# Ighina/MultimodalTopicSegmentation

Measured on NVIDIA B200. Metric: segmented sentences/sec, higher is better.
Workload: dtype f32

## Files before the change

multimodaltopicsegmentation_b200/csrc/lstm_rec_h3.cu:

```cuda
#include <cooperative_groups.h>
#include <cuda_fp16.h>
#include <stdlib.h>

#include "cluster_utils.cuh"
#include "tcgen05_utils.cuh"

namespace cg = cooperative_groups;

namespace mts {

constexpr int HR_NB = 16;
constexpr int HR_SUB_THREADS = 160;
constexpr int HR_EPI = 128;
constexpr int HR_PIECE_BYTES = 4 * HR_NB * 128;
constexpr int HR_B_BYTES = 2 * HR_PIECE_BYTES;
constexpr int HR_ACT_FLOATS = 4 * HR_NB * 32;
constexpr int HR_TMEM_COLS = 512;
constexpr int HR_W2_COL = 128;
constexpr int HR_ACC_COL = 256;
constexpr int HR_SUB_BYTES = 2 * HR_B_BYTES + HR_ACT_FLOATS * 4 + 1024;
constexpr int HR_HEAD_BYTES = 1024;
static_assert(HR_SUB_BYTES % 1024 == 0, "SWIZZLE_128B operand buffers need 1024-byte alignment");
template <int NT>
constexpr int hr_smem() {
  return (HR_HEAD_BYTES + NT * HR_SUB_BYTES + 1024) > 120 * 1024 ? (HR_HEAD_BYTES + NT * HR_SUB_BYTES + 1024) : 120 * 1024;
}

__host__ __device__ constexpr uint32_t idesc_f16(int M, int N) {
  return (1u << 4) | ((uint32_t)(N >> 3) << 17) | ((uint32_t)(M >> 4) << 24);
}

__device__ __forceinline__ uint32_t h2_bits(float first, float second) {
  const __half2 h = __floats2half2_rn(first, second);
  return *reinterpret_cast<const uint32_t *>(&h);
}
__device__ __forceinline__ float2 h2_floats(uint32_t bits) {
  return __half22float2(*reinterpret_cast<const __half2 *>(&bits));
}
__device__ __forceinline__ void st_async_v4u(uint32_t raddr, uint4 v, uint32_t rbar) {
  asm volatile("st.async.weak.shared::cluster.mbarrier::complete_tx::bytes.v4.b32 [%0], {%1, %2, %3, %4}, [%5];" ::"r"(raddr),
               "r"(v.x), "r"(v.y), "r"(v.z), "r"(v.w), "r"(rbar)
               : "memory");
}
__device__ __forceinline__ void tmem_st16u(uint32_t taddr, const uint32_t (&v)[16]) {
  asm volatile(
      "tcgen05.st.sync.aligned.32x32b.x16.b32 [%0], "
      "{%1, %2, %3, %4, %5, %6, %7, %8, %9, %10, %11, %12, %13, %14, %15, %16};" ::"r"(taddr),
      "r"(v[0]), "r"(v[1]), "r"(v[2]), "r"(v[3]), "r"(v[4]), "r"(v[5]), "r"(v[6]), "r"(v[7]), "r"(v[8]), "r"(v[9]), "r"(v[10]),
      "r"(v[11]), "r"(v[12]), "r"(v[13]), "r"(v[14]), "r"(v[15])
      : "memory");
}

__device__ __forceinline__ void umma_f16_ts_p(uint32_t d_tmem, uint32_t a_tmem, uint32_t b_lo, uint32_t b_hi, uint32_t idesc,
                                              uint32_t acc) {
  asm volatile(
      "{\n\t.reg .pred p;\n\t.reg .b64 bd;\n\t"
      "setp.ne.b32 p, %5, 0;\n\t"
      "mov.b64 bd, {%2, %3};\n\t"
      "tcgen05.mma.cta_group::1.kind::f16 [%0], [%1], bd, %4, p;\n\t}" ::"r"(d_tmem),
      "r"(a_tmem), "r"(b_lo), "r"(b_hi), "r"(idesc), "r"(acc)
      : "memory");
}

constexpr int HR_PROF_STEPS = 4, HR_PROF_SLOTS = 16;
__device__ long long *g_hr_prof = nullptr;
#define HR_STAMP(slot)                                                                     \
  do {                                                                                     \
    if (prof && s >= 8 && s < 8 + HR_PROF_STEPS) prof[(s - 8) * HR_PROF_SLOTS + (slot)] = clock64(); \
  } while (0)

template <bool SAVE, int NT, bool BF16>
__global__ void __cluster_dims__(kCluster, 1, 1) __launch_bounds__(HR_SUB_THREADS * NT, 1)
    lstm_fwd_h3_kernel(const float *__restrict__ gx, const float *__restrict__ w_hh, const int32_t *__restrict__ lengths,
                       const int32_t *__restrict__ order, int B, int T, int n_enc, int n_tiles, int ept,
                       float *__restrict__ y, float *__restrict__ gates, float *__restrict__ y_corr) {
  constexpr bool bf16_mode = BF16;
  extern __shared__ uint8_t smem_raw[];
  uint8_t *smem = reinterpret_cast<uint8_t *>((reinterpret_cast<uintptr_t>(smem_raw) + 1023) & ~(uintptr_t)1023);
  const int tid = threadIdx.x, lane = tid & 31;
  const int warp = __shfl_sync(0xffffffffu, tid >> 5, 0);
  const int sub = (NT == 2 && warp >= 5) ? 1 : 0;
  const int wr = warp - 5 * sub;

  float *rscale_s = reinterpret_cast<float *>(smem);
  uint32_t *tmem_slot = reinterpret_cast<uint32_t *>(smem + 512);
  uint8_t *sub_base = smem + HR_HEAD_BYTES + sub * HR_SUB_BYTES;
  uint8_t *bbuf = sub_base;
  float *act = reinterpret_cast<float *>(bbuf + 2 * HR_B_BYTES);
  uint64_t *bars = reinterpret_cast<uint64_t *>(act + HR_ACT_FLOATS);
  uint64_t *h_full = bars;
  uint64_t *acc_full = bars + 16;
  int *len_s = reinterpret_cast<int *>(bars + 18);
  int *bq_s = len_s + HR_NB;

  cg::cluster_group cluster = cg::this_cluster();
  const uint32_t rank = cluster.block_rank();
  const int n_clusters = gridDim.x / kCluster;
  const int groups = (n_tiles + NT - 1) / NT;
  const int n_items = groups * 2 * n_enc;
  const int ycols = n_enc * 2 * kH;

  if (wr == 0 && lane == 0) {
    for (int i = 0; i < 4; ++i) tc::bar_init(tc::s_u32(&h_full[i]), 1);
    tc::bar_init(tc::s_u32(acc_full), 1);
    asm volatile("fence.mbarrier_init.release.cluster;" ::: "memory");
  }
  if (warp == 0) tc::tmem_alloc<HR_TMEM_COLS>(tc::s_u32(tmem_slot));
  tc::tc_fence_before();
  __syncthreads();
  tc::tc_fence_after();
  const uint32_t tmem_base = *tmem_slot;
  const uint32_t acc_col = HR_ACC_COL + 16 * sub;

  uint32_t ph_h = 0, ph_acc = 0;

  const int et = (wr - 1) * 32 + lane;
  const int q = warp & 3;
  const int cj = et & 7, ce = et >> 3;

  int cur_dir = -1, cur_enc = -1;
  long long *prof = (blockIdx.x == 0 && (tid == 0 || tid == 32)) ? g_hr_prof : nullptr;

  for (int item = blockIdx.x / kCluster; item < n_items; item += n_clusters) {
    const int tile = (item % groups) * NT + sub;
    const int dir = (item / groups) & 1;
    const int enc = item / (2 * groups);
    const float *W = w_hh + ((size_t)enc * 2 + dir) * 4 * kH * kH;

    if (dir != cur_dir || enc != cur_enc) {
      if (sub == 0 && wr >= 1) {
        const float *wrow = W + (size_t)(q * kH + rank * kUnits + lane) * kH;
        float mx = 0.0f;
#pragma unroll 8
        for (int i = 0; i < kH / 4; ++i) {
          const float4 x = __ldg(reinterpret_cast<const float4 *>(wrow) + i);
          mx = fmaxf(fmaxf(mx, fmaxf(fabsf(x.x), fabsf(x.y))), fmaxf(fabsf(x.z), fabsf(x.w)));
        }
        const int ex = (int)((__float_as_uint(mx) >> 23) & 0xFFu);
        int sexp = ex == 0 ? 0 : 127 + 13 - ex;
        sexp = sexp > 110 ? 110 : sexp;
        const float sc = __uint_as_float((uint32_t)(127 + sexp) << 23);
        rscale_s[q * 32 + lane] = __uint_as_float((uint32_t)(127 - sexp) << 23);
        const uint32_t trow = tmem_base + ((uint32_t)(q * 32) << 16);
#pragma unroll 1
        for (int kk = 0; kk < 8; ++kk) {
          const int src_blk = ((int)rank - kk) & 7;
          uint32_t w1[16], w2[16];
#pragma unroll
          for (int i = 0; i < 8; ++i) {
            const float4 x = __ldg(reinterpret_cast<const float4 *>(wrow + src_blk * 32) + i);
            const float a = x.x * sc, b = x.y * sc, c = x.z * sc, d = x.w * sc;
            if (bf16_mode) {
              w1[2 * i] = bf16x2_bits(a, b);
              w1[2 * i + 1] = bf16x2_bits(c, d);
              w2[2 * i] = w2[2 * i + 1] = 0u;
            } else {
              w1[2 * i] = h2_bits(a, b);
              w1[2 * i + 1] = h2_bits(c, d);
              const float2 f0 = h2_floats(w1[2 * i]), f1 = h2_floats(w1[2 * i + 1]);
              w2[2 * i] = h2_bits(a - f0.x, b - f0.y);
              w2[2 * i + 1] = h2_bits(c - f1.x, d - f1.y);
            }
          }
          tmem_st16u(trow + (uint32_t)(kk * 16), w1);
          tmem_st16u(trow + (uint32_t)(HR_W2_COL + kk * 16), w2);
        }
        tc::tmem_wait_st();
      }
      cur_dir = dir;
      cur_enc = enc;
    }
    const int st = tid - sub * HR_SUB_THREADS;
    if (st < HR_NB) {
      const int slot = tile * ept + st;
      const int bq = (tile < n_tiles && st < ept && slot < B) ? (order ? order[slot] : slot) : -1;
      bq_s[st] = bq;
      len_s[st] = (bq >= 0) ? min(max(lengths[bq], 0), T) : 0;
    }
    for (int idx = st; idx < 2 * HR_B_BYTES / 16; idx += HR_SUB_THREADS)
      reinterpret_cast<float4 *>(bbuf)[idx] = make_float4(0.f, 0.f, 0.f, 0.f);
    tc::fence_proxy_async();
    tc::tc_fence_before();
    __syncthreads();
    tc::tc_fence_after();
    int nsteps = 0;
#pragma unroll
    for (int e = 0; e < HR_NB; ++e) nsteps = max(nsteps, len_s[e]);
    cluster.sync();

    const size_t gx_enc = (size_t)enc * B * T * 8 * kH;

    if (wr == 0) {
      constexpr uint32_t idesc = bf16_mode ? tc::idesc_bf16(128, HR_NB) : idesc_f16(128, HR_NB);
      const uint32_t tb = __shfl_sync(0xffffffffu, tmem_base, 0);
      const uint32_t d_tmem = tb + acc_col;
      const bool leader = tc::elect_one();
      const uint64_t dfull = tc::desc_sw128(tc::s_u32(bbuf));
      const uint32_t dlo0 = __shfl_sync(0xffffffffu, (uint32_t)dfull, 0), dhi = (uint32_t)(dfull >> 32);
      const uint32_t half_tx = (uint32_t)(4 * ept * (bf16_mode ? 64 : 128));
      for (int s = 0; s < nsteps; ++s) {
        const int p = s & 1;
        HR_STAMP(0);
        if (leader && s + 1 < nsteps) {
          tc::bar_expect_tx(tc::s_u32(&h_full[(p ^ 1) * 2 + 0]), half_tx);
          tc::bar_expect_tx(tc::s_u32(&h_full[(p ^ 1) * 2 + 1]), half_tx);
        }
        const uint32_t dlo = dlo0 + (uint32_t)(p * (HR_B_BYTES >> 4));
#pragma unroll
        for (int g = 0; g < 2; ++g) {
          if (s > 0) tc::bar_wait_wd(tc::s_u32(&h_full[p * 2 + g]), (ph_h >> p) & 1u);
          HR_STAMP(1 + g);
          tc::tc_fence_after();
          if (leader) {
#pragma unroll
            for (int i = 4 * g; i < 4 * g + 4; ++i) {
#pragma unroll
              for (int k = 0; k < 2; ++k) {
                const uint32_t d1 = dlo + (uint32_t)(((i >> 1) * (HR_NB * 128) + (i & 1) * 64 + k * 32) >> 4);
                const uint32_t d2 = d1 + (uint32_t)(HR_PIECE_BYTES >> 4);
                const uint32_t a1 = tb + (uint32_t)(16 * i + 8 * k), a2 = a1 + HR_W2_COL;
                umma_f16_ts_p(d_tmem, a1, d1, dhi, idesc, (i | k) != 0);
                if (!bf16_mode) {
                  umma_f16_ts_p(d_tmem, a2, d1, dhi, idesc, 1);
                  umma_f16_ts_p(d_tmem, a1, d2, dhi, idesc, 1);
                }
              }
            }
          }
          HR_STAMP(3 + g);
        }
        if (s > 0) ph_h ^= 1u << p;
        if (leader) tc::umma_commit(tc::s_u32(acc_full));
        __syncwarp();
        HR_STAMP(5);
      }
    } else {
      const int gcol = dir * 4 * kH + q * kH + (int)rank * kUnits + lane;
      const float rs = rscale_s[q * 32 + lane];
      float gxn[HR_NB];
#pragma unroll
      for (int e = 0; e < HR_NB; ++e) {
        const int len = len_s[e];
        gxn[e] = 0.0f;
        if (len > 0) {
          const int t0 = dir ? len - 1 : 0;
          gxn[e] = __ldg(gx + gx_enc + ((size_t)bq_s[e] * T + t0) * 8 * kH + gcol);
        }
      }
      float c[4] = {0.f, 0.f, 0.f, 0.f};
      const int my_len = len_s[ce], my_b = bq_s[ce];
      const size_t ycol = (size_t)enc * 2 * kH + dir * kH + rank * kUnits + 4 * cj;
      const size_t gate_base = ((size_t)enc * 2 + dir) * B;
      const int piece = cj & 1, chunk = cj >> 1;
      uint32_t raddr[kCluster], rbar[kCluster];
#pragma unroll
      for (int i = 0; i < kCluster; ++i) {
        const uint32_t r = (rank + i) & 7;
        const uint32_t off = (uint32_t)(piece * HR_PIECE_BYTES + (i >> 1) * (HR_NB * 128) + ce * 128 +
                                        ((((i & 1) * 4 + chunk) ^ (ce & 7)) << 4));
        raddr[i] = mapa(tc::s_u32(bbuf) + off, r);
        rbar[i] = mapa(tc::s_u32(&h_full[i >> 2]), r);
      }
      const bool sender = ce < ept && !(bf16_mode && piece);

      for (int s = 0; s < nsteps; ++s) {
        const int p = s & 1;
        float gxc[HR_NB];
#pragma unroll
        for (int e = 0; e < HR_NB; ++e) {
          gxc[e] = gxn[e];
          const int len = len_s[e];
          if (s + 1 < len) {
            const int tn = dir ? len - 2 - s : s + 1;
            gxn[e] = __ldg(gx + gx_enc + ((size_t)bq_s[e] * T + tn) * 8 * kH + gcol);
          }
        }
        tc::bar_wait_wd(tc::s_u32(acc_full), ph_acc); ph_acc ^= 1;
        HR_STAMP(10);
        tc::tc_fence_after();
        float pre[HR_NB];
        tc::tmem_ld16(tmem_base + ((uint32_t)(q * 32) << 16) + acc_col, pre);
        tc::tc_fence_before();
        HR_STAMP(11);
        const float zs = (q == 2) ? -2.0f * 1.4426950408889634f : -1.4426950408889634f;
        const float oa = (q == 2) ? 2.0f : 1.0f, ob = (q == 2) ? -1.0f : 0.0f;
#define HR_ACT(NCOL)                                                          \
  _Pragma("unroll") for (int e = 0; e < (NCOL); ++e) {                        \
    const float z = fmaf(pre[e], rs, gxc[e]);                                 \
    const float sg = __fdividef(1.0f, 1.0f + exp2f(z * zs));                  \
    act[(q * HR_NB + e) * 32 + lane] = fmaf(sg, oa, ob);                      \
  }
        if (ept > 14) { HR_ACT(16) } else if (ept > 12) { HR_ACT(14) } else if (ept > 10) { HR_ACT(12) } else if (ept > 8) { HR_ACT(10) }
        else if (ept > 6) { HR_ACT(8) } else if (ept > 4) { HR_ACT(6) } else if (ept > 2) { HR_ACT(4) } else { HR_ACT(2) }
#undef HR_ACT
        if (sub == 0) asm volatile("bar.sync 1, 128;" ::: "memory");
        else asm volatile("bar.sync 2, 128;" ::: "memory");
        HR_STAMP(12);
        const float4 ig = *reinterpret_cast<const float4 *>(act + (0 * HR_NB + ce) * 32 + 4 * cj);
        const float4 fg = *reinterpret_cast<const float4 *>(act + (1 * HR_NB + ce) * 32 + 4 * cj);
        const float4 gg = *reinterpret_cast<const float4 *>(act + (2 * HR_NB + ce) * 32 + 4 * cj);
        const float4 og = *reinterpret_cast<const float4 *>(act + (3 * HR_NB + ce) * 32 + 4 * cj);
        float4 hn = make_float4(0.f, 0.f, 0.f, 0.f);
        if (s < my_len) {
          c[0] = fmaf(fg.x, c[0], ig.x * gg.x); c[1] = fmaf(fg.y, c[1], ig.y * gg.y);
          c[2] = fmaf(fg.z, c[2], ig.z * gg.z); c[3] = fmaf(fg.w, c[3], ig.w * gg.w);
          hn = make_float4(og.x * tanh_fast(c[0]), og.y * tanh_fast(c[1]), og.z * tanh_fast(c[2]), og.w * tanh_fast(c[3]));
        }
        HR_STAMP(13);
        if (s + 1 < nsteps) {
          uint32_t p1a, p1b, p2a = 0u, p2b = 0u;
          if (bf16_mode) {
            p1a = bf16x2_bits(hn.x, hn.y);
            p1b = bf16x2_bits(hn.z, hn.w);
          } else {
            p1a = h2_bits(hn.x, hn.y);
            p1b = h2_bits(hn.z, hn.w);
            const float2 f0 = h2_floats(p1a), f1 = h2_floats(p1b);
            p2a = h2_bits(hn.x - f0.x, hn.y - f0.y);
            p2b = h2_bits(hn.z - f1.x, hn.w - f1.y);
          }
          const uint32_t ga = piece ? p1a : p2a, gb = piece ? p1b : p2b;
          const uint32_t ra = __shfl_xor_sync(0xffffffffu, ga, 1), rb = __shfl_xor_sync(0xffffffffu, gb, 1);
          const uint4 gran = piece ? make_uint4(ra, rb, p2a, p2b) : make_uint4(p1a, p1b, ra, rb);
          if (sender) {
            const uint32_t boff = (uint32_t)((p ^ 1) * HR_B_BYTES), moff = (uint32_t)((p ^ 1) * 16);
#pragma unroll
            for (int r = 0; r < kCluster; ++r) st_async_v4u(raddr[r] + boff, gran, rbar[r] + moff);
          }
        }
        HR_STAMP(14);
        if (s < my_len) {
          const int t = dir ? my_len - 1 - s : s;
          *reinterpret_cast<float4 *>(y + ((size_t)my_b * T + t) * ycols + ycol) = hn;
          if (y_corr) corr_store4(y_corr + ((size_t)my_b * T + t) * ycols, (int)ycol, hn, 0);
          if (SAVE) {
            float *gs = gates + ((gate_base + my_b) * T + t) * 5 * kH + rank * kUnits + 4 * cj;
            *reinterpret_cast<float4 *>(gs) = ig;
            *reinterpret_cast<float4 *>(gs + kH) = fg;
            *reinterpret_cast<float4 *>(gs + 2 * kH) = gg;
            *reinterpret_cast<float4 *>(gs + 3 * kH) = og;
            *reinterpret_cast<float4 *>(gs + 4 * kH) = make_float4(c[0], c[1], c[2], c[3]);
          }
        }
      }
      if (my_b >= 0)
        for (int t = my_len; t < T; ++t) {
          const float4 z = make_float4(0.f, 0.f, 0.f, 0.f);
          *reinterpret_cast<float4 *>(y + ((size_t)my_b * T + t) * ycols + ycol) = z;
          if (y_corr) corr_store4(y_corr + ((size_t)my_b * T + t) * ycols, (int)ycol, z, 0);
        }
    }
    tc::tc_fence_before();
    __syncthreads();
    cluster.sync();
  }
  tc::tc_fence_before();
  __syncthreads();
  if (warp == 0) {
    tc::tc_fence_after();
    tc::tmem_dealloc<HR_TMEM_COLS>(tmem_base);
  }
}

template <typename K>
static int h3_max_active_clusters(K kernel, int threads, int smem) {
  cudaLaunchConfig_t cfg = {};
  cfg.gridDim = dim3(kCluster * 64);
  cfg.blockDim = dim3(threads);
  cfg.dynamicSmemBytes = smem;
  cudaLaunchAttribute attr;
  attr.id = cudaLaunchAttributeClusterDimension;
  attr.val.clusterDim.x = kCluster;
  attr.val.clusterDim.y = 1;
  attr.val.clusterDim.z = 1;
  cfg.attrs = &attr;
  cfg.numAttrs = 1;
  int n = 0;
  if (cudaOccupancyMaxActiveClusters(&n, kernel, &cfg) != cudaSuccess || n < 1) {
    cudaGetLastError();
    n = 8;
  }
  return n;
}

}

using namespace mts;

extern "C" int mts_debug_rec_profile_h3(long long *buf) {
  MTS_CUDA(cudaMemcpyToSymbol(g_hr_prof, &buf, sizeof(buf)));
  return 0;
}

template <bool BF16>
static int launch_h3(const float *gx, const float *w_hh, const int32_t *lengths, const int32_t *order, int n_enc, int B, int T,
                     float *y, float *gates, float *y_corr, cudaStream_t st) {
  MTS_PER_DEVICE(int, cap);
  if (!cap) {
    MTS_CUDA(cudaFuncSetAttribute(lstm_fwd_h3_kernel<false, 1, BF16>, cudaFuncAttributeMaxDynamicSharedMemorySize, hr_smem<1>()));
    MTS_CUDA(cudaFuncSetAttribute(lstm_fwd_h3_kernel<true, 1, BF16>, cudaFuncAttributeMaxDynamicSharedMemorySize, hr_smem<1>()));
    MTS_CUDA(cudaFuncSetAttribute(lstm_fwd_h3_kernel<false, 2, BF16>, cudaFuncAttributeMaxDynamicSharedMemorySize, hr_smem<2>()));
    MTS_CUDA(cudaFuncSetAttribute(lstm_fwd_h3_kernel<true, 2, BF16>, cudaFuncAttributeMaxDynamicSharedMemorySize, hr_smem<2>()));
    cap = h3_max_active_clusters(lstm_fwd_h3_kernel<false, 2, BF16>, 2 * HR_SUB_THREADS, hr_smem<2>());
  }
  int ept = HR_NB;
  {
    const int per_dir = cap / (2 * n_enc);
    if (per_dir >= 1 && (B + HR_NB - 1) / HR_NB <= per_dir) {
      const int want = (B + per_dir - 1) / per_dir;
      ept = want < 1 ? 1 : (want > HR_NB ? HR_NB : want);
    }
  }
  static const char *force_ept = getenv("MTS_REC_EPT");
  if (force_ept && atoi(force_ept) >= 1 && atoi(force_ept) <= HR_NB) ept = atoi(force_ept);
  const int n_tiles = (B + ept - 1) / ept;
  const int items1 = n_tiles * 2 * n_enc;
  static const char *force = getenv("MTS_REC_NT");
  const bool two = force ? (force[0] == '2') : (items1 > cap);
  static const char *pair_env = getenv("MTS_REC_PAIR");
  if (pair_env ? (pair_env[0] == '1') : two)
    return mts_lstm_rec_fwd_h3p(gx, w_hh, lengths, order, n_enc, B, T, kH, y, gates, y_corr, BF16 ? 1 : 0, (void *)st);
  if (!two) {
    const unsigned grid = (unsigned)((items1 < cap ? items1 : cap) * kCluster);
    if (gates) lstm_fwd_h3_kernel<true, 1, BF16><<<grid, HR_SUB_THREADS, hr_smem<1>(), st>>>(gx, w_hh, lengths, order, B, T, n_enc, n_tiles, ept, y, gates, y_corr);
    else lstm_fwd_h3_kernel<false, 1, BF16><<<grid, HR_SUB_THREADS, hr_smem<1>(), st>>>(gx, w_hh, lengths, order, B, T, n_enc, n_tiles, ept, y, gates, y_corr);
  } else {
    const int items2 = ((n_tiles + 1) / 2) * 2 * n_enc;
    const unsigned grid = (unsigned)((items2 < cap ? items2 : cap) * kCluster);
    if (gates) lstm_fwd_h3_kernel<true, 2, BF16><<<grid, 2 * HR_SUB_THREADS, hr_smem<2>(), st>>>(gx, w_hh, lengths, order, B, T, n_enc, n_tiles, ept, y, gates, y_corr);
    else lstm_fwd_h3_kernel<false, 2, BF16><<<grid, 2 * HR_SUB_THREADS, hr_smem<2>(), st>>>(gx, w_hh, lengths, order, B, T, n_enc, n_tiles, ept, y, gates, y_corr);
  }
  MTS_LAUNCH_CHECK();
  return 0;
}

extern "C" int mts_lstm_rec_fwd_h3(const float *gx, const float *w_hh, const int32_t *lengths, const int32_t *order, int n_enc,
                                   int B, int T, int H, float *y, float *gates, float *y_corr, int precision, void *stream) {
  MTS_REQUIRE(gx && w_hh && lengths && y, MTS_E_BADARG, "lstm_rec_fwd_h3: null pointer");
  MTS_REQUIRE(n_enc >= 1 && B > 0 && T > 0, MTS_E_BADARG, "lstm_rec_fwd_h3: bad shape");
  MTS_REQUIRE(H == kH, MTS_E_UNSUPPORTED, "lstm_rec_fwd_h3: the tensor-core recurrence serves H == 256");
  MTS_REQUIRE(precision == 0 || precision == 1, MTS_E_BADARG, "lstm_rec_fwd_h3: precision must be 0 (fp16 x3) or 1 (bf16)");
  MTS_REQUIRE(!y_corr || n_enc == 1, MTS_E_UNSUPPORTED, "lstm_rec_fwd_h3: the fused correction operand needs n_enc == 1");
  MTS_REQUIRE((((uintptr_t)y | (uintptr_t)gx | (uintptr_t)w_hh) & 15) == 0, MTS_E_BADARG,
              "lstm_rec_fwd_h3: buffers must be 16-byte aligned");
  cudaStream_t st = (cudaStream_t)stream;
  return precision ? launch_h3<true>(gx, w_hh, lengths, order, n_enc, B, T, y, gates, y_corr, st)
                   : launch_h3<false>(gx, w_hh, lengths, order, n_enc, B, T, y, gates, y_corr, st);
}
```

Measured before the change: 18.58 million.

## Split LSTM recurrence epilogue across eight warps for single-tile pipeline

Adds an eight-warp epilogue variant in which each group of four warps handles half of the batch columns. It loads eight TMEM columns instead of sixteen and remaps the cell-update lanes across the larger warp set, which shortens the per-step serial activation and cell-update work on the recurrence's critical path. The variant is used in the single-tile path whenever there are at least three elements per tile, or when forced by an environment variable. In exchange the block is larger and uses a wider named barrier, and the column interleave adds indexing complexity.

```diff
diff --git a/multimodaltopicsegmentation_b200/csrc/lstm_rec_h3.cu b/multimodaltopicsegmentation_b200/csrc/lstm_rec_h3.cu
--- a/multimodaltopicsegmentation_b200/csrc/lstm_rec_h3.cu
+++ b/multimodaltopicsegmentation_b200/csrc/lstm_rec_h3.cu
@@ -10,8 +10,7 @@
 namespace mts {
 
 constexpr int HR_NB = 16;
-constexpr int HR_SUB_THREADS = 160;
-constexpr int HR_EPI = 128;
+constexpr int HR_EPI8_MIN_EPT = 3;
 constexpr int HR_PIECE_BYTES = 4 * HR_NB * 128;
 constexpr int HR_B_BYTES = 2 * HR_PIECE_BYTES;
 constexpr int HR_ACT_FLOATS = 4 * HR_NB * 32;
@@ -42,6 +41,20 @@
                "r"(v.x), "r"(v.y), "r"(v.z), "r"(v.w), "r"(rbar)
                : "memory");
 }
+__device__ __forceinline__ void tmem_ld8(uint32_t taddr, float (&v)[8]) {
+  uint32_t r[8];
+  asm volatile("tcgen05.ld.sync.aligned.32x32b.x8.b32 {%0, %1, %2, %3, %4, %5, %6, %7}, [%8];"
+               : "=r"(r[0]), "=r"(r[1]), "=r"(r[2]), "=r"(r[3]), "=r"(r[4]), "=r"(r[5]), "=r"(r[6]), "=r"(r[7])
+               : "r"(taddr)
+               : "memory");
+  asm volatile("tcgen05.wait::ld.sync.aligned;" ::: "memory");
+#pragma unroll
+  for (int i = 0; i < 8; ++i) v[i] = __uint_as_float(r[i]);
+}
+template <int HALVES>
+__device__ __forceinline__ int hr_col(int e) {
+  return (e % HALVES) * (HR_NB / HALVES) + e / HALVES;
+}
 __device__ __forceinline__ void tmem_st16u(uint32_t taddr, const uint32_t (&v)[16]) {
   asm volatile(
       "tcgen05.st.sync.aligned.32x32b.x16.b32 [%0], "
@@ -69,18 +82,22 @@
     if (prof && s >= 8 && s < 8 + HR_PROF_STEPS) prof[(s - 8) * HR_PROF_SLOTS + (slot)] = clock64(); \
   } while (0)
 
-template <bool SAVE, int NT, bool BF16>
-__global__ void __cluster_dims__(kCluster, 1, 1) __launch_bounds__(HR_SUB_THREADS * NT, 1)
+template <bool SAVE, int NT, bool BF16, int EW>
+__global__ void __cluster_dims__(kCluster, 1, 1) __launch_bounds__(32 * (1 + EW) * NT, 1)
     lstm_fwd_h3_kernel(const float *__restrict__ gx, const float *__restrict__ w_hh, const int32_t *__restrict__ lengths,
                        const int32_t *__restrict__ order, int B, int T, int n_enc, int n_tiles, int ept,
                        float *__restrict__ y, float *__restrict__ gates, float *__restrict__ y_corr) {
+  static_assert(EW == 4 || (EW == 8 && NT == 1), "eight epilogue warps only with one tile pipeline");
   constexpr bool bf16_mode = BF16;
+  constexpr int SUBT = 32 * (1 + EW);
+  constexpr int HALVES = EW / 4;
+  constexpr int CPW = HR_NB / HALVES;
   extern __shared__ uint8_t smem_raw[];
   uint8_t *smem = reinterpret_cast<uint8_t *>((reinterpret_cast<uintptr_t>(smem_raw) + 1023) & ~(uintptr_t)1023);
   const int tid = threadIdx.x, lane = tid & 31;
   const int warp = __shfl_sync(0xffffffffu, tid >> 5, 0);
-  const int sub = (NT == 2 && warp >= 5) ? 1 : 0;
-  const int wr = warp - 5 * sub;
+  const int sub = (NT == 2 && warp > EW) ? 1 : 0;
+  const int wr = warp - (1 + EW) * sub;
 
   float *rscale_s = reinterpret_cast<float *>(smem);
   uint32_t *tmem_slot = reinterpret_cast<uint32_t *>(smem + 512);
@@ -114,9 +131,8 @@
 
   uint32_t ph_h = 0, ph_acc = 0;
 
-  const int et = (wr - 1) * 32 + lane;
   const int q = warp & 3;
-  const int cj = et & 7, ce = et >> 3;
+  const int col0 = ((wr - 1) >> 2) * CPW;
 
   int cur_dir = -1, cur_enc = -1;
   long long *prof = (blockIdx.x == 0 && (tid == 0 || tid == 32)) ? g_hr_prof : nullptr;
@@ -128,7 +144,7 @@
     const float *W = w_hh + ((size_t)enc * 2 + dir) * 4 * kH * kH;
 
     if (dir != cur_dir || enc != cur_enc) {
-      if (sub == 0 && wr >= 1) {
+      if (sub == 0 && wr >= 1 && wr <= 4) {
         const float *wrow = W + (size_t)(q * kH + rank * kUnits + lane) * kH;
         float mx = 0.0f;
 #pragma unroll 8
@@ -170,14 +186,14 @@
       cur_dir = dir;
       cur_enc = enc;
     }
-    const int st = tid - sub * HR_SUB_THREADS;
+    const int st = tid - sub * SUBT;
     if (st < HR_NB) {
       const int slot = tile * ept + st;
       const int bq = (tile < n_tiles && st < ept && slot < B) ? (order ? order[slot] : slot) : -1;
-      bq_s[st] = bq;
-      len_s[st] = (bq >= 0) ? min(max(lengths[bq], 0), T) : 0;
+      bq_s[hr_col<HALVES>(st)] = bq;
+      len_s[hr_col<HALVES>(st)] = (bq >= 0) ? min(max(lengths[bq], 0), T) : 0;
     }
-    for (int idx = st; idx < 2 * HR_B_BYTES / 16; idx += HR_SUB_THREADS)
+    for (int idx = st; idx < 2 * HR_B_BYTES / 16; idx += SUBT)
       reinterpret_cast<float4 *>(bbuf)[idx] = make_float4(0.f, 0.f, 0.f, 0.f);
     tc::fence_proxy_async();
     tc::tc_fence_before();
@@ -237,49 +253,54 @@
     } else {
       const int gcol = dir * 4 * kH + q * kH + (int)rank * kUnits + lane;
       const float rs = rscale_s[q * 32 + lane];
-      float gxn[HR_NB];
-#pragma unroll
-      for (int e = 0; e < HR_NB; ++e) {
-        const int len = len_s[e];
+      float gxn[CPW];
+#pragma unroll
+      for (int e = 0; e < CPW; ++e) {
+        const int len = len_s[col0 + e];
         gxn[e] = 0.0f;
         if (len > 0) {
           const int t0 = dir ? len - 1 : 0;
-          gxn[e] = __ldg(gx + gx_enc + ((size_t)bq_s[e] * T + t0) * 8 * kH + gcol);
+          gxn[e] = __ldg(gx + gx_enc + ((size_t)bq_s[col0 + e] * T + t0) * 8 * kH + gcol);
         }
       }
+      const int piece = lane & 1, chunk = (lane >> 1) & 3, cj = 2 * chunk + piece;
+      const int ce = (lane >> 3) * EW + ((wr - 1 - chunk * ept) & (EW - 1));
+      const bool cell = ce < ept;
+      const int row = cell ? hr_col<HALVES>(ce) : 0;
       float c[4] = {0.f, 0.f, 0.f, 0.f};
-      const int my_len = len_s[ce], my_b = bq_s[ce];
+      const int my_len = cell ? len_s[row] : 0, my_b = cell ? bq_s[row] : -1;
       const size_t ycol = (size_t)enc * 2 * kH + dir * kH + rank * kUnits + 4 * cj;
       const size_t gate_base = ((size_t)enc * 2 + dir) * B;
-      const int piece = cj & 1, chunk = cj >> 1;
       uint32_t raddr[kCluster], rbar[kCluster];
 #pragma unroll
       for (int i = 0; i < kCluster; ++i) {
         const uint32_t r = (rank + i) & 7;
-        const uint32_t off = (uint32_t)(piece * HR_PIECE_BYTES + (i >> 1) * (HR_NB * 128) + ce * 128 +
-                                        ((((i & 1) * 4 + chunk) ^ (ce & 7)) << 4));
+        const uint32_t off = (uint32_t)(piece * HR_PIECE_BYTES + (i >> 1) * (HR_NB * 128) + row * 128 +
+                                        ((((i & 1) * 4 + chunk) ^ (row & 7)) << 4));
         raddr[i] = mapa(tc::s_u32(bbuf) + off, r);
         rbar[i] = mapa(tc::s_u32(&h_full[i >> 2]), r);
       }
-      const bool sender = ce < ept && !(bf16_mode && piece);
+      const bool sender = cell && !(bf16_mode && piece);
+      const int ncol = (ept + HALVES - 1 - col0 / CPW) / HALVES;
 
       for (int s = 0; s < nsteps; ++s) {
         const int p = s & 1;
-        float gxc[HR_NB];
-#pragma unroll
-        for (int e = 0; e < HR_NB; ++e) {
+        float gxc[CPW];
+#pragma unroll
+        for (int e = 0; e < CPW; ++e) {
           gxc[e] = gxn[e];
-          const int len = len_s[e];
+          const int len = len_s[col0 + e];
           if (s + 1 < len) {
             const int tn = dir ? len - 2 - s : s + 1;
-            gxn[e] = __ldg(gx + gx_enc + ((size_t)bq_s[e] * T + tn) * 8 * kH + gcol);
+            gxn[e] = __ldg(gx + gx_enc + ((size_t)bq_s[col0 + e] * T + tn) * 8 * kH + gcol);
           }
         }
         tc::bar_wait_wd(tc::s_u32(acc_full), ph_acc); ph_acc ^= 1;
         HR_STAMP(10);
         tc::tc_fence_after();
-        float pre[HR_NB];
-        tc::tmem_ld16(tmem_base + ((uint32_t)(q * 32) << 16) + acc_col, pre);
+        float pre[CPW];
+        if constexpr (CPW == 16) tc::tmem_ld16(tmem_base + ((uint32_t)(q * 32) << 16) + acc_col, pre);
+        else tmem_ld8(tmem_base + ((uint32_t)(q * 32) << 16) + acc_col + col0, pre);
         tc::tc_fence_before();
         HR_STAMP(11);
         const float zs = (q == 2) ? -2.0f * 1.4426950408889634f : -1.4426950408889634f;
@@ -288,20 +309,24 @@
   _Pragma("unroll") for (int e = 0; e < (NCOL); ++e) {                        \
     const float z = fmaf(pre[e], rs, gxc[e]);                                 \
     const float sg = __fdividef(1.0f, 1.0f + exp2f(z * zs));                  \
-    act[(q * HR_NB + e) * 32 + lane] = fmaf(sg, oa, ob);                      \
-  }
-        if (ept > 14) { HR_ACT(16) } else if (ept > 12) { HR_ACT(14) } else if (ept > 10) { HR_ACT(12) } else if (ept > 8) { HR_ACT(10) }
-        else if (ept > 6) { HR_ACT(8) } else if (ept > 4) { HR_ACT(6) } else if (ept > 2) { HR_ACT(4) } else { HR_ACT(2) }
+    act[(q * HR_NB + col0 + e) * 32 + lane] = fmaf(sg, oa, ob);               \
+  }
+        if constexpr (CPW == 16) {
+          if (ncol > 14) { HR_ACT(16) } else if (ncol > 12) { HR_ACT(14) } else if (ncol > 10) { HR_ACT(12) } else if (ncol > 8) { HR_ACT(10) }
+          else if (ncol > 6) { HR_ACT(8) } else if (ncol > 4) { HR_ACT(6) } else if (ncol > 2) { HR_ACT(4) } else { HR_ACT(2) }
+        } else {
+          if (ncol > 6) { HR_ACT(8) } else if (ncol > 4) { HR_ACT(6) } else if (ncol > 2) { HR_ACT(4) } else if (ncol > 0) { HR_ACT(2) }
+        }
 #undef HR_ACT
-        if (sub == 0) asm volatile("bar.sync 1, 128;" ::: "memory");
-        else asm volatile("bar.sync 2, 128;" ::: "memory");
+        asm volatile("bar.sync %0, %1;" ::"r"(1 + sub), "n"(32 * EW) : "memory");
         HR_STAMP(12);
-        const float4 ig = *reinterpret_cast<const float4 *>(act + (0 * HR_NB + ce) * 32 + 4 * cj);
-        const float4 fg = *reinterpret_cast<const float4 *>(act + (1 * HR_NB + ce) * 32 + 4 * cj);
-        const float4 gg = *reinterpret_cast<const float4 *>(act + (2 * HR_NB + ce) * 32 + 4 * cj);
-        const float4 og = *reinterpret_cast<const float4 *>(act + (3 * HR_NB + ce) * 32 + 4 * cj);
+        float4 ig, fg, gg, og;
         float4 hn = make_float4(0.f, 0.f, 0.f, 0.f);
         if (s < my_len) {
+          ig = *reinterpret_cast<const float4 *>(act + (0 * HR_NB + row) * 32 + 4 * cj);
+          fg = *reinterpret_cast<const float4 *>(act + (1 * HR_NB + row) * 32 + 4 * cj);
+          gg = *reinterpret_cast<const float4 *>(act + (2 * HR_NB + row) * 32 + 4 * cj);
+          og = *reinterpret_cast<const float4 *>(act + (3 * HR_NB + row) * 32 + 4 * cj);
           c[0] = fmaf(fg.x, c[0], ig.x * gg.x); c[1] = fmaf(fg.y, c[1], ig.y * gg.y);
           c[2] = fmaf(fg.z, c[2], ig.z * gg.z); c[3] = fmaf(fg.w, c[3], ig.w * gg.w);
           hn = make_float4(og.x * tanh_fast(c[0]), og.y * tanh_fast(c[1]), og.z * tanh_fast(c[2]), og.w * tanh_fast(c[3]));
@@ -397,11 +422,13 @@
                      float *y, float *gates, float *y_corr, cudaStream_t st) {
   MTS_PER_DEVICE(int, cap);
   if (!cap) {
-    MTS_CUDA(cudaFuncSetAttribute(lstm_fwd_h3_kernel<false, 1, BF16>, cudaFuncAttributeMaxDynamicSharedMemorySize, hr_smem<1>()));
-    MTS_CUDA(cudaFuncSetAttribute(lstm_fwd_h3_kernel<true, 1, BF16>, cudaFuncAttributeMaxDynamicSharedMemorySize, hr_smem<1>()));
-    MTS_CUDA(cudaFuncSetAttribute(lstm_fwd_h3_kernel<false, 2, BF16>, cudaFuncAttributeMaxDynamicSharedMemorySize, hr_smem<2>()));
-    MTS_CUDA(cudaFuncSetAttribute(lstm_fwd_h3_kernel<true, 2, BF16>, cudaFuncAttributeMaxDynamicSharedMemorySize, hr_smem<2>()));
-    cap = h3_max_active_clusters(lstm_fwd_h3_kernel<false, 2, BF16>, 2 * HR_SUB_THREADS, hr_smem<2>());
+    MTS_CUDA(cudaFuncSetAttribute(lstm_fwd_h3_kernel<false, 1, BF16, 4>, cudaFuncAttributeMaxDynamicSharedMemorySize, hr_smem<1>()));
+    MTS_CUDA(cudaFuncSetAttribute(lstm_fwd_h3_kernel<true, 1, BF16, 4>, cudaFuncAttributeMaxDynamicSharedMemorySize, hr_smem<1>()));
+    MTS_CUDA(cudaFuncSetAttribute(lstm_fwd_h3_kernel<false, 1, BF16, 8>, cudaFuncAttributeMaxDynamicSharedMemorySize, hr_smem<1>()));
+    MTS_CUDA(cudaFuncSetAttribute(lstm_fwd_h3_kernel<true, 1, BF16, 8>, cudaFuncAttributeMaxDynamicSharedMemorySize, hr_smem<1>()));
+    MTS_CUDA(cudaFuncSetAttribute(lstm_fwd_h3_kernel<false, 2, BF16, 4>, cudaFuncAttributeMaxDynamicSharedMemorySize, hr_smem<2>()));
+    MTS_CUDA(cudaFuncSetAttribute(lstm_fwd_h3_kernel<true, 2, BF16, 4>, cudaFuncAttributeMaxDynamicSharedMemorySize, hr_smem<2>()));
+    cap = h3_max_active_clusters(lstm_fwd_h3_kernel<false, 2, BF16, 4>, 2 * 32 * 5, hr_smem<2>());
   }
   int ept = HR_NB;
   {
@@ -422,13 +449,20 @@
     return mts_lstm_rec_fwd_h3p(gx, w_hh, lengths, order, n_enc, B, T, kH, y, gates, y_corr, BF16 ? 1 : 0, (void *)st);
   if (!two) {
     const unsigned grid = (unsigned)((items1 < cap ? items1 : cap) * kCluster);
-    if (gates) lstm_fwd_h3_kernel<true, 1, BF16><<<grid, HR_SUB_THREADS, hr_smem<1>(), st>>>(gx, w_hh, lengths, order, B, T, n_enc, n_tiles, ept, y, gates, y_corr);
-    else lstm_fwd_h3_kernel<false, 1, BF16><<<grid, HR_SUB_THREADS, hr_smem<1>(), st>>>(gx, w_hh, lengths, order, B, T, n_enc, n_tiles, ept, y, gates, y_corr);
+    const char *epi_env = getenv("MTS_REC_EPI");
+    const bool eight = epi_env ? (epi_env[0] == '8') : (ept >= HR_EPI8_MIN_EPT);
+    if (eight) {
+      if (gates) lstm_fwd_h3_kernel<true, 1, BF16, 8><<<grid, 32 * 9, hr_smem<1>(), st>>>(gx, w_hh, lengths, order, B, T, n_enc, n_tiles, ept, y, gates, y_corr);
+      else lstm_fwd_h3_kernel<false, 1, BF16, 8><<<grid, 32 * 9, hr_smem<1>(), st>>>(gx, w_hh, lengths, order, B, T, n_enc, n_tiles, ept, y, gates, y_corr);
+    } else {
+      if (gates) lstm_fwd_h3_kernel<true, 1, BF16, 4><<<grid, 32 * 5, hr_smem<1>(), st>>>(gx, w_hh, lengths, order, B, T, n_enc, n_tiles, ept, y, gates, y_corr);
+      else lstm_fwd_h3_kernel<false, 1, BF16, 4><<<grid, 32 * 5, hr_smem<1>(), st>>>(gx, w_hh, lengths, order, B, T, n_enc, n_tiles, ept, y, gates, y_corr);
+    }
   } else {
     const int items2 = ((n_tiles + 1) / 2) * 2 * n_enc;
     const unsigned grid = (unsigned)((items2 < cap ? items2 : cap) * kCluster);
-    if (gates) lstm_fwd_h3_kernel<true, 2, BF16><<<grid, 2 * HR_SUB_THREADS, hr_smem<2>(), st>>>(gx, w_hh, lengths, order, B, T, n_enc, n_tiles, ept, y, gates, y_corr);
-    else lstm_fwd_h3_kernel<false, 2, BF16><<<grid, 2 * HR_SUB_THREADS, hr_smem<2>(), st>>>(gx, w_hh, lengths, order, B, T, n_enc, n_tiles, ept, y, gates, y_corr);
+    if (gates) lstm_fwd_h3_kernel<true, 2, BF16, 4><<<grid, 2 * 32 * 5, hr_smem<2>(), st>>>(gx, w_hh, lengths, order, B, T, n_enc, n_tiles, ept, y, gates, y_corr);
+    else lstm_fwd_h3_kernel<false, 2, BF16, 4><<<grid, 2 * 32 * 5, hr_smem<2>(), st>>>(gx, w_hh, lengths, order, B, T, n_enc, n_tiles, ept, y, gates, y_corr);
   }
   MTS_LAUNCH_CHECK();
   return 0;
```

After: 15.88 million (median of 6 runs). 0.854x the previous value.
